# PJLab-ADG/neuralsim

Hardware: AMD Instinct MI355X
Metric: training rays/sec (fwd+bwd) NeuS 800x800 (higher is better)
Workload: dtype fp16

## Files before the change

neuralsim_amd/csrc/field.hip:

```cpp
#include "lotd_dev.h"
#include "mfma_mlp.h"
#include "occ_dev.h"
#include <stdlib.h>

enum { M_W1 = 0, M_W2, M_W2T, M_W1T, M_R1, M_R2, M_R3, M_R3T, M_R2T, M_R1T, M_COUNT };
enum { V_B1 = 0, V_B2, V_WH, V_RB1, V_RB2, V_RB3, V_SCAL, V_COUNT };

struct FieldLayout {
  int64_t mat[M_COUNT];
  int64_t vec[V_COUNT];
  int64_t vend;
  int64_t mat16[4];
  int64_t total;
  int elt;
  int split;
};

static const int kMatUo[M_COUNT] = {64, 64, 64, 32, 64, 64, 32, 64, 64, 32};
static const int kMatUi[M_COUNT] = {32, 64, 64, 64, 32, 64, 64, 32, 64, 64};

static inline int mat_uo(int m, int nc) { return m == M_W1T ? 32 * nc : kMatUo[m]; }
static inline int mat_ui(int m, int nc) { return m == M_W1 ? 32 * nc : kMatUi[m]; }
static inline int field_nc(int num_levels) { return num_levels > 16 ? 2 : 1; }
static inline int field_ne(const NsimFieldMeta* meta) { return meta->embed_E > 0 ? 2 : 0; }
// ... 439 lines not shown
#pragma unroll
        for (int b = 0; b < 2; ++b) {
          const int l = 4 * q + 2 * hi + b, r0 = 4 * q + 2 * b;
          const float* hp = reinterpret_cast<const float*>(pf + 256 * l) + 2 * j;
          h[r0] = valid ? hp[0] : 0.f;
          h[r0 + 1] = valid ? hp[1] : 0.f;
        }
      nsim_wait_lgkm0();
      p = load_point(a, tile, j, true);
      const int64_t sc = valid ? s : a.S - 1;
#pragma unroll
      for (int q = 0; q < 4; ++q)
#pragma unroll
        for (int b = 0; b < 2; ++b) {
          const int l = 4 * q + 2 * hi + b, r0 = 4 * q + 2 * b;
          const JPair<JT>* jp = reinterpret_cast<const JPair<JT>*>(reinterpret_cast<const JT*>(a.J_pl) + ((int64_t)l * a.PS + sc) * 6);
          Jq[2 * q + b][0] = jp[0];
          Jq[2 * q + b][1] = jp[1];
          Jq[2 * q + b][2] = jp[2];
        }
      if (tile + wstride < ntiles) prefetch_planes(tile + wstride);
    } else if constexpr (GLDS) {
      nsim_wait_vm0();
#pragma unroll
      for (int m = 0; m < NC; ++m)
#pragma unroll
      for (int q = 0; q < 4; ++q)
#pragma unroll
        for (int b = 0; b < 2; ++b) {
          const int l = 16 * m + 4 * q + 2 * hi + b, r0 = 16 * m + 4 * q + 2 * b;
          const float* hp = reinterpret_cast<const float*>(pf + 1024 * l) + 2 * j;
          const JT* jp = reinterpret_cast<const JT*>(pf + 1024 * l + 256) + 6 * j;
          const bool lv = valid && LV_OK(l);
          h[r0] = lv ? hp[0] : 0.f;
          h[r0 + 1] = lv ? hp[1] : 0.f;
          float ja[3], jb[3];
          jload6(jp, ja, jb);
#pragma unroll
          for (int c3 = 0; c3 < 3; ++c3) {
            J[r0][c3] = lv ? ja[c3] : 0.f;
            J[r0 + 1][c3] = lv ? jb[c3] : 0.f;
          }
        }
      nsim_wait_lgkm0();
      if (tile + wstride < ntiles) prefetch_planes(tile + wstride);
    } else if constexpr (FROM_PLANES) {
#pragma unroll
      for (int m = 0; m < NC; ++m)
#pragma unroll
        for (int q = 0; q < 4; ++q)
#pragma unroll
          for (int b = 0; b < 2; ++b) {
            const int l = 16 * m + 4 * q + 2 * hi + b;
            const int r0 = 16 * m + 4 * q + 2 * b;
            h[r0] = h[r0 + 1] = 0.f;
            if (valid && LV_OK(l)) {
              const float* hp = a.h_pl + ((int64_t)l * a.PS + s) * 2;
              h[r0] = hp[0];
              h[r0 + 1] = hp[1];
            }
          }
      if constexpr (NC == 1 && NE == 0) {
#pragma unroll
        for (int q = 0; q < 4; ++q)
#pragma unroll
          for (int b = 0; b < 2; ++b) {
            const int l = 4 * q + 2 * hi + b;
            const int r0 = 4 * q + 2 * b;
#pragma unroll
            for (int c3 = 0; c3 < 3; ++c3) J[r0][c3] = J[r0 + 1][c3] = 0.f;
            if (valid && LV_OK(l)) {
              jload6(reinterpret_cast<const JT*>(a.J_pl) + ((int64_t)l * a.PS + s) * 6, J[r0], J[r0 + 1]);
            }
          }
      }
    } else if constexpr (NC == 1) {
#pragma unroll
      for (int q = 0; q < 4; ++q) {
#pragma unroll
        for (int b = 0; b < 2; ++b) {
          const int l = 4 * q + 2 * hi + b;
          const LotdRes R = a.lotd.res[l];
          const LotdCell c = lotd_cell(p.xx, R, a.lotd);
          float f0 = 0.f, f1 = 0.f, j0[3] = {0.f, 0.f, 0.f}, j1[3] = {0.f, 0.f, 0.f};
          const int pm = lotd_slot_mask(c);
          if (l < a.lotd.n_active)
#pragma unroll
          for (int slot = 0; slot < 8; ++slot) {
            const int corner = slot ^ pm;
            float w, dw[3];
            lotd_corner_w(c, corner, w, dw);
            const uint32_t idx = lotd_index(c.c0[0] + (corner & 1), c.c0[1] + ((corner >> 1) & 1),
                                            c.c0[2] + ((corner >> 2) & 1), R, a.lotd.type[l], a.lotd.size[l]);
            float g0, g1;
            lotd_load2(gref, (uint32_t)a.lotd.offset[l] + p.goff + 2u * idx, g0, g1);
            f0 = f0 + w * g0;
            f1 = f1 + w * g1;
#pragma unroll
            for (int c3 = 0; c3 < 3; ++c3) {
              j0[c3] = j0[c3] + dw[c3] * g0;
              j1[c3] = j1[c3] + dw[c3] * g1;
            }
          }
          const int r0 = 4 * q + 2 * b;
          h[r0] = f0;
          h[r0 + 1] = f1;
#pragma unroll
          for (int c3 = 0; c3 < 3; ++c3) {
            J[r0][c3] = j0[c3] * c.dscale[c3];
            J[r0 + 1][c3] = j1[c3] * c.dscale[c3];
          }
          if (a.h_pl && valid) {
            float* hp = a.h_pl + ((int64_t)l * a.PS + s) * 2;
            JT* jp = reinterpret_cast<JT*>(a.J_pl) + ((int64_t)l * a.PS + s) * 6;
            hp[0] = f0;
            hp[1] = f1;
            jstore6(jp, J[r0], J[r0 + 1]);
          }
        }
      }
    }
    if constexpr (NE > 0) embed_eval(a, p.xx, valid, hi, reinterpret_cast<float(&)[32]>(h[16 * NC]), ed);
    float a1[32];
    dense<PREC, 2, NI>(a1, W + L.mat[M_W1], h, true);
#pragma unroll
    for (int k = 0; k < 32; ++k) a1[k] = softplus_b(a1[k] + vecf(W, L, V_B1, hi, k), beta, inv_beta);
    float a2[32];
    if constexpr (SDF_D == 2) {
      dense<PREC, 2, 2>(a2, W + L.mat[M_W2], a1, false);
#pragma unroll
      for (int k = 0; k < 32; ++k) a2[k] = softplus_b(a2[k] + vecf(W, L, V_B2, hi, k), beta, inv_beta);
    } else {
#pragma unroll
      for (int k = 0; k < 32; ++k) a2[k] = a1[k];
    }
    float sdf = 0.f;
#pragma unroll
    for (int k = 0; k < 32; ++k) sdf = sdf + vecf(W, L, V_WH, hi, k) * a2[k];
    sdf = sdf + wave_shfl_xor(sdf, 32);
    sdf = sdf + b_out;
    float e1[32];
    float d1[32];
    if constexpr (SDF_D == 2) {
      float d2[32];
#pragma unroll
      for (int k = 0; k < 32; ++k) d2[k] = sig_from_softplus(a2[k], beta) * vecf(W, L, V_WH, hi, k);
      dense<PREC, 2, 2>(e1, W + L.mat[M_W2T], d2, false);
#pragma unroll
      for (int k = 0; k < 32; ++k) d1[k] = sig_from_softplus(a1[k], beta) * e1[k];
    } else {
#pragma unroll
      for (int k = 0; k < 32; ++k) {
        e1[k] = vecf(W, L, V_WH, hi, k);
        d1[k] = sig_from_softplus(a1[k], beta) * e1[k];
      }
    }
    float g[16 * NI];
    dense<PREC, NI, 2>(g, W + L.mat[M_W1T], d1, false);
    float nab[3];
    if constexpr (JDIR) {
      float acc[3] = {0.f, 0.f, 0.f};
#pragma unroll
      for (int e = 0; e < 8; ++e) {
        const int r0 = 4 * (e >> 1) + 2 * (e & 1);
        acc[0] = acc[0] + g[r0] * (float)Jq[e][0].x + g[r0 + 1] * (float)Jq[e][1].y;
        acc[1] = acc[1] + g[r0] * (float)Jq[e][0].y + g[r0 + 1] * (float)Jq[e][2].x;
        acc[2] = acc[2] + g[r0] * (float)Jq[e][1].x + g[r0 + 1] * (float)Jq[e][2].y;
      }
#pragma unroll
      for (int c3 = 0; c3 < 3; ++c3) nab[c3] = acc[c3] + wave_shfl_xor(acc[c3], 32);
    } else if constexpr ((NC == 1 && NE == 0) || GL2) {
#pragma unroll
      for (int c3 = 0; c3 < 3; ++c3) {
        float acc = 0.f;
#pragma unroll
        for (int f = 0; f < 16 * NC; ++f) acc = acc + g[f] * J[f][c3];
        nab[c3] = acc + wave_shfl_xor(acc, 32);
      }
    } else {
      float acc[3] = {0.f, 0.f, 0.f};
      if (valid) {
#pragma unroll
        for (int m = 0; m < NC; ++m)
#pragma unroll
          for (int q = 0; q < 4; ++q)
// ... 591 lines not shown
        dz1[k] = gs * wh * s1 + dh1[k] * wh * (beta * s1 * (1.0f - s1));
      }
    }
    bh += wave_sum(g == 0 ? gs : 0.f);
    __syncthreads();
    jstage16<4>(stA, dz1, wave);
    jstage16<2>(stB, h, wave);
    if constexpr (SDF_D == 1) jstage16<4>(stC, whv, wave);
    __syncthreads();
    if (do_dw) {
      jdw16_tiles<2>(stA, wave, stB, 0, accW1, &bs1);
      if constexpr (SDF_D == 1) bsh += j16_row_share(stC, wave);
    }
    float dh[8];
    dense16<2, 4>(dh, W + L.mat16[M_W1T], dz1, true);
    if (a.dx) {
      float acc[3] = {0.f, 0.f, 0.f};
      if (valid) {
#pragma unroll
        for (int m = 0; m < 2; ++m)
#pragma unroll
          for (int b = 0; b < 2; ++b) {
            const int l = 8 * m + 2 * g + b, r0 = 4 * m + 2 * b;
            float ja[3], jb[3];
            jload6(reinterpret_cast<const JT*>(a.J_pl) + ((int64_t)l * a.PS + s) * 6, ja, jb);
#pragma unroll
            for (int c3 = 0; c3 < 3; ++c3) acc[c3] = acc[c3] + dh[r0] * ja[c3] + dh[r0 + 1] * jb[c3];
          }
      }
#pragma unroll
      for (int c3 = 0; c3 < 3; ++c3) {
        acc[c3] = acc[c3] + wave_shfl_xor(acc[c3], 16);
        acc[c3] = acc[c3] + wave_shfl_xor(acc[c3], 32);
      }
      if (valid && g == 0) {
#pragma unroll
        for (int c3 = 0; c3 < 3; ++c3) a.dx[3 * s + c3] = a.dx[3 * s + c3] + acc[c3];
      }
    }
    if (valid && a.dh_pl) {
#pragma unroll
      for (int m = 0; m < 2; ++m)
#pragma unroll
        for (int b = 0; b < 2; ++b) {
          const int l = 8 * m + 2 * g + b, r0 = 4 * m + 2 * b;
          float* dp = a.dh_pl + ((int64_t)l * a.S + s) * 2;
          dp[0] = dh[r0];
          dp[1] = dh[r0 + 1];
        }
    }
  }
  const int F1 = 2 * a.lotd.num_levels;
  const SrcOff so = src_off(SDF_D, F1);
  const int64_t ro = (int64_t)(blockIdx.x & (unsigned)a.rep_mask) * a.rep_stride;
#pragma unroll
  for (int n = 0; n < 2; ++n) jflush16(a.dsdf_w + ro + so.w1, F1, F1, wave, n, accW1[n]);
  bs1 += wave_shfl_xor(bs1, 16);
  bs1 += wave_shfl_xor(bs1, 32);
  bsh += wave_shfl_xor(bsh, 16);
  bsh += wave_shfl_xor(bsh, 32);
  if constexpr (SDF_D == 2) {
#pragma unroll
    for (int n = 0; n < 4; ++n) jflush16(a.dsdf_w + ro + so.w2, 64, 64, wave, n, accW2[n]);
    bs2 += wave_shfl_xor(bs2, 16);
    bs2 += wave_shfl_xor(bs2, 32);
    if (g == 0 && bs2 != 0.f) atomicAdd(&a.dsdf_b[ro + so.b2 + 16 * wave + p], bs2);
  }
  if (g == 0 && bs1 != 0.f) atomicAdd(&a.dsdf_b[ro + so.b1 + 16 * wave + p], bs1);
  if (g == 0 && bsh != 0.f) atomicAdd(&a.dsdf_w[ro + so.wh + 16 * wave + p], bsh);
  if (lane == 0 && bh != 0.f) atomicAdd(&a.dsdf_b[ro + so.bh], bh);
}

#define SDF_H_SCALE 1024.0f
#ifndef NSIM_SDF_MIN_WAVES
#define NSIM_SDF_MIN_WAVES 2
#endif
constexpr int GLM_PTS = 2;
constexpr int GLM_PTS_WJ = 1;
template <int PREC, bool WJ>
__global__ void __launch_bounds__(64, 1) k_lotd_gather_lm(FieldArgs a) {
  using JT = typename JPlane<PREC>::T;
  constexpr int NP = WJ ? GLM_PTS_WJ : GLM_PTS;
  const int lane = nsim_lane();
  const int xcd = (int)(blockIdx.x & 7u);
  const int64_t s0 = (int64_t)(blockIdx.x >> 3) * (64 * NP) + lane;
  int64_t Sv = a.S;
  if (a.S_dev) {
    const int64_t sd = a.S_dev[0] + a.S_add;
    Sv = sd <= Sv ? sd : 0;
  }
  if (s0 - lane >= Sv) return;
  float xx[NP][3];
  uint32_t goff[NP];
#pragma unroll
  for (int q = 0; q < NP; ++q) {
    const int64_t s = s0 + 64 * q;
    xx[q][0] = xx[q][1] = xx[q][2] = 0.f;
    goff[q] = 0u;
    if (s < Sv) {
      if (a.ray_goff) goff[q] = (uint32_t)a.ray_goff[a.ridx[s]];
      if (a.x) {
        xx[q][0] = a.x[3 * s]; xx[q][1] = a.x[3 * s + 1]; xx[q][2] = a.x[3 * s + 2];
      } else {
        const int64_t ray = a.ridx[s];
        const float tt = a.t[s];
#pragma unroll
        for (int c = 0; c < 3; ++c) xx[q][c] = a.rays_o[3 * ray + c] + tt * a.rays_d[3 * ray + c];
      }
    }
  }
  const GridRef gref = grid_ref(a.grid);
  const int nl = a.glm_n[xcd];
  const int64_t nblk_valid = (Sv + 64 * NP - 1) / (64 * NP);
  const bool second_half = (int64_t)(blockIdx.x >> 3) >= (nblk_valid + 1) / 2;
#pragma unroll 1
  for (int k = 0; k < nl; ++k) {
    const int l = a.glm_lv[xcd][k];
    const int half = a.glm_half[xcd][k];
    if ((half == 1 && second_half) || (half == 2 && !second_half)) continue;
    const LotdRes R = a.lotd.res[l];
    const int type = a.lotd.type[l];
    const uint32_t T = a.lotd.size[l], off = (uint32_t)a.lotd.offset[l];
    float f0[NP], f1[NP];
    float j0[WJ ? NP : 1][3], j1[WJ ? NP : 1][3];
#pragma unroll
    for (int q = 0; q < NP; ++q) {
      const LotdCell c = lotd_cell(xx[q], R, a.lotd);
      f0[q] = f1[q] = 0.f;
      if constexpr (WJ) {
#pragma unroll
        for (int c3 = 0; c3 < 3; ++c3) j0[q][c3] = j1[q][c3] = 0.f;
      }
      constexpr bool SLOTS = WJ;
      const LotdSlots SL = lotd_slots(c);
      const int pm = lotd_slot_mask(c);
      if (l < a.lotd.n_active)
#pragma unroll
      for (int slot = 0; slot < 8; ++slot) {
        float w, dw[3];
        uint32_t idx;
        if constexpr (SLOTS) {
          lotd_slot_w(SL, slot, w, dw);
          idx = lotd_slot_index(SL, slot, R, type, T);
        } else {
          const int corner = slot ^ pm;
          lotd_corner_w(c, corner, w, dw);
          idx = lotd_index(c.c0[0] + (corner & 1), c.c0[1] + ((corner >> 1) & 1), c.c0[2] + ((corner >> 2) & 1), R, type, T);
        }
        float g0, g1;
        lotd_load2(gref, off + goff[q] + 2u * idx, g0, g1);
        f0[q] = f0[q] + w * g0;
        f1[q] = f1[q] + w * g1;
        if constexpr (WJ) {
#pragma unroll
          for (int c3 = 0; c3 < 3; ++c3) {
            j0[q][c3] = j0[q][c3] + dw[c3] * g0;
            j1[q][c3] = j1[q][c3] + dw[c3] * g1;
          }
        }
      }
      if constexpr (WJ) {
#pragma unroll
        for (int c3 = 0; c3 < 3; ++c3) {
          j0[q][c3] = j0[q][c3] * c.dscale[c3];
          j1[q][c3] = j1[q][c3] * c.dscale[c3];
        }
      }
    }
#pragma unroll
    for (int q = 0; q < NP; ++q) {
      const int64_t s = s0 + 64 * q;
      if (s < Sv) {
        const int64_t e = (int64_t)l * a.PS + s;
        if constexpr (WJ) {
          const int64_t ep = (int64_t)l * a.PS + s;
          float* hp = a.h_pl + ep * 2;
          JT* jp = reinterpret_cast<JT*>(a.J_pl) + ep * 6;
          hp[0] = f0[q];
          hp[1] = f1[q];
          jstore6(jp, j0[q], j1[q]);
        } else if constexpr (PREC == 0) {
          union {
            uint32_t u;
            f16 h[2];
          } cv;
          cv.h[0] = (f16)f16_sat(f0[q] * SDF_H_SCALE);
          cv.h[1] = (f16)f16_sat(f1[q] * SDF_H_SCALE);
          reinterpret_cast<uint32_t*>(a.feat_pl)[e] = cv.u;
        } else {
          reinterpret_cast<float*>(a.feat_pl)[2 * e] = f0[q];
          reinterpret_cast<float*>(a.feat_pl)[2 * e + 1] = f1[q];
        }
      }
    }
  }
}

template <int PREC, bool WJ>
static void launch_gather_lm(const FieldArgs& a, int64_t S, hipStream_t stream) {
  const dim3 gg((unsigned)(8 * nsim_blocks(S, 64 * (WJ ? GLM_PTS_WJ : GLM_PTS))));
  hipLaunchKernelGGL((k_lotd_gather_lm<PREC, WJ>), gg, dim3(64), 0, stream, a);
}

__device__ __forceinline__ void sdf_gather8(const FieldArgs& a, const GridRef& gref, const TilePoint& p, int lb, int hi,
                                            float (&f8)[8]) {
#pragma unroll
  for (int qq = 0; qq < 2; ++qq) {
#pragma unroll
    for (int b = 0; b < 2; ++b) {
      const int l = lb + 4 * qq + 2 * hi + b;
      const LotdRes R = a.lotd.res[l];
      const LotdCell c = lotd_cell(p.xx, R, a.lotd);
      float f0 = 0.f, f1 = 0.f;
      const int pm = lotd_slot_mask(c);
      if (l < a.lotd.n_active)
#pragma unroll
      for (int slot = 0; slot < 8; ++slot) {
        const int corner = slot ^ pm;
        float w, dw[3];
        lotd_corner_w(c, corner, w, dw);
        const uint32_t idx = lotd_index(c.c0[0] + (corner & 1), c.c0[1] + ((corner >> 1) & 1),
                                        c.c0[2] + ((corner >> 2) & 1), R, a.lotd.type[l], a.lotd.size[l]);
        float g0, g1;
        lotd_load2(gref, (uint32_t)a.lotd.offset[l] + p.goff + 2u * idx, g0, g1);
        f0 = f0 + w * g0;
        f1 = f1 + w * g1;
      }
      f8[4 * qq + 2 * b] = f0;
      f8[4 * qq + 2 * b + 1] = f1;
    }
  }
}

template <int PREC, int NC, bool HAVE_BV>
__device__ __forceinline__ void sdf_layer1_step(const char* W, const FieldLayout& L, int rb, int lane, const float (&f8)[8],
                                                const f16x8& bvp, f32x16 (&acc)[2], f32x16 (&accc)[PREC == 2 ? 2 : 1]) {
  constexpr bool PLANES = HAVE_BV;
  if constexpr (PREC == 0) {
    f16x8 bv;
    if constexpr (PLANES) {
      bv = bvp;
    } else {
#pragma unroll
      for (int e = 0; e < 8; ++e) bv[e] = (f16)f16_sat(f8[e] * SDF_H_SCALE);
    }
    const f16x8* A = reinterpret_cast<const f16x8*>(W + L.mat[M_W1]);
#pragma unroll
    for (int mo = 0; mo < 2; ++mo) acc[mo] = mfma_32x32x16_f16(A[(mo * 2 * NC + rb) * 64 + lane], bv, acc[mo]);
  } else if constexpr (PREC == 2) {
    f16x8 bh, bl;
#pragma unroll
    for (int e = 0; e < 8; ++e) {
      f16 h_, l_;
      split_f16(f8[e] * SDF_H_SCALE, h_, l_);
      bh[e] = h_;
      bl[e] = l_;
    }
    const f16x8* Ah = reinterpret_cast<const f16x8*>(W + L.mat[M_W1]);
    const f16x8* Al = Ah + 64 * 4 * NC;
#pragma unroll
    for (int mo = 0; mo < 2; ++mo) {
      const int fi = (mo * 2 * NC + rb) * 64 + lane;
      acc[mo] = mfma_32x32x16_f16(Ah[fi], bh, acc[mo]);
      accc[mo] = mfma_32x32x16_f16(Ah[fi], bl, accc[mo]);
      accc[mo] = mfma_32x32x16_f16(Al[fi], bh, accc[mo]);
    }
  } else {
    const float* A = reinterpret_cast<const float*>(W + L.mat[M_W1]);
#pragma unroll
    for (int e = 0; e < 8; ++e)
#pragma unroll
      for (int mo = 0; mo < 2; ++mo)
        acc[mo] = mfma_32x32x2_f32(A[(mo * 16 * NC + 8 * rb + e) * 64 + lane], f8[e], acc[mo]);
  }
}

template <int PREC, int SDF_D>
__device__ __forceinline__ float sdf_decode(const char* W, const FieldLayout& L, f32x16 (&acc)[2],
                                            f32x16 (&accc)[PREC == 2 ? 2 : 1], int hi, int lane, float beta, float inv_beta,
                                            float b_out) {
  const float inv_h = PREC != 1 ? 1.0f / SDF_H_SCALE : 1.0f;
  float sdf = 0.f;
  if constexpr (PREC == 2) {
#pragma unroll
    for (int mo = 0; mo < 2; ++mo)
#pragma unroll
      for (int r = 0; r < 16; ++r) acc[mo][r] = acc[mo][r] + accc[mo][r] * (1.0f / SPLIT_LO_SCALE);
  }
  if constexpr (PREC == 2 && SDF_D == 2) {
    f16x8 bqh[4], bql[4];
#pragma unroll
    for (int mo = 0; mo < 2; ++mo)
#pragma unroll
      for (int r = 0; r < 16; ++r) {
        f16 h_, l_;
        split_f16(softplus_exact(acc[mo][r] * inv_h + vecf(W, L, V_B1, hi, mo * 16 + r), beta, inv_beta), h_, l_);
        bqh[2 * mo + (r >> 3)][r & 7] = h_;
        bql[2 * mo + (r >> 3)][r & 7] = l_;
      }
    const f16x8* A2h = reinterpret_cast<const f16x8*>(W + L.mat[M_W2]);
    const f16x8* A2l = A2h + 64 * 8;
#pragma unroll
    for (int mo = 0; mo < 2; ++mo) {
      f32x16 acc2 = zero16(), acc2c = zero16();
#pragma unroll
      for (int st = 0; st < 4; ++st) {
        const int fi = (mo * 4 + st) * 64 + lane;
        acc2 = mfma_32x32x16_f16(A2h[fi], bqh[st], acc2);
        acc2c = mfma_32x32x16_f16(A2h[fi], bql[st], acc2c);
        acc2c = mfma_32x32x16_f16(A2l[fi], bqh[st], acc2c);
      }
#pragma unroll
// ... 1326 lines not shown
```

neuralsim_amd/csrc/lotd.hip:

```cpp
#include "lotd_dev.h"

__global__ void __launch_bounds__(256) k_lotd_fwd(const float* __restrict__ x, const f16* __restrict__ grid,
                                                   LotdDev m, int64_t S, float* __restrict__ out,
                                                   float* __restrict__ dydx) {
  const int64_t tid = (int64_t)blockIdx.x * blockDim.x + threadIdx.x;
  const int L = m.num_levels;
  if (tid >= S * L) return;
  const int64_t s = tid / L;
  const int l = (int)(tid % L);
  const float xx[3] = {x[3 * s], x[3 * s + 1], x[3 * s + 2]};
  const LotdRes R = m.res[l];
  const LotdCell c = lotd_cell(xx, R, m);
  float f0 = 0.f, f1 = 0.f;
  float j0[3] = {0.f, 0.f, 0.f}, j1[3] = {0.f, 0.f, 0.f};
  const int pm = lotd_slot_mask(c);
  if (l < m.n_active)
#pragma unroll
  for (int slot = 0; slot < 8; ++slot) {
    const int corner = slot ^ pm;
    float w, dw[3];
    lotd_corner_w(c, corner, w, dw);
    const uint32_t idx = lotd_index(c.c0[0] + (corner & 1), c.c0[1] + ((corner >> 1) & 1),
                                    c.c0[2] + ((corner >> 2) & 1), R, m.type[l], m.size[l]);
    float g0, g1;
    lotd_load2(grid, m.offset[l], idx, g0, g1);
    f0 = f0 + w * g0;
    f1 = f1 + w * g1;
    if (dydx) {
#pragma unroll
      for (int a = 0; a < 3; ++a) {
        j0[a] = j0[a] + dw[a] * g0;
        j1[a] = j1[a] + dw[a] * g1;
      }
    }
  }
  const int64_t o = s * (2 * L) + 2 * l;
  out[o] = f0;
  out[o + 1] = f1;
  if (dydx) {
#pragma unroll
    for (int a = 0; a < 3; ++a) {
      dydx[o * 3 + a] = j0[a] * c.dscale[a];
      dydx[(o + 1) * 3 + a] = j1[a] * c.dscale[a];
    }
  }
}

__global__ void __launch_bounds__(256) k_lotd_bwd(const float* __restrict__ x, const float* __restrict__ dout,
                                                   const float* __restrict__ ddydx, LotdDev m, int64_t S,
                                                   float* __restrict__ dgrid) {
  const int64_t tid = (int64_t)blockIdx.x * blockDim.x + threadIdx.x;
  const int L = m.num_levels;
  if (tid >= S * L) return;
  const int64_t s = tid / L;
  const int l = (int)(tid % L);
  if (l >= m.n_active) return;
  const float xx[3] = {x[3 * s], x[3 * s + 1], x[3 * s + 2]};
  const LotdRes R = m.res[l];
  const LotdCell c = lotd_cell(xx, R, m);
  const int64_t o = s * (2 * L) + 2 * l;
  const float d0 = dout ? dout[o] : 0.f, d1 = dout ? dout[o + 1] : 0.f;
  float q0[3] = {0.f, 0.f, 0.f}, q1[3] = {0.f, 0.f, 0.f};
  if (ddydx) {
#pragma unroll
    for (int a = 0; a < 3; ++a) {
      q0[a] = ddydx[o * 3 + a] * c.dscale[a];
      q1[a] = ddydx[(o + 1) * 3 + a] * c.dscale[a];
    }
  }
#pragma unroll
  for (int corner = 0; corner < 8; ++corner) {
    float w, dw[3];
    lotd_corner_w(c, corner, w, dw);
    const uint32_t idx = lotd_index(c.c0[0] + (corner & 1), c.c0[1] + ((corner >> 1) & 1),
                                    c.c0[2] + ((corner >> 2) & 1), R, m.type[l], m.size[l]);
    const float v0 = w * d0 + (dw[0] * q0[0] + dw[1] * q0[1] + dw[2] * q0[2]);
    const float v1 = w * d1 + (dw[0] * q1[0] + dw[1] * q1[1] + dw[2] * q1[2]);
    float* dst = dgrid + m.offset[l] + 2 * (int64_t)idx;
    if (v0 != 0.f) atomicAdd(dst, v0);
    if (v1 != 0.f) atomicAdd(dst + 1, v1);
  }
}

extern "C" {

int nsim_lotd_fwd(const float* x, const void* grid_f16, const NsimLotdMeta* meta, int64_t S, float* out,
                  float* dydx, void* stream) {
  const int rc = lotd_meta_check(meta);
  if (rc) return rc;
  if (S <= 0) return 0;
  hipLaunchKernelGGL(k_lotd_fwd, dim3(nsim_blocks(S * meta->num_levels, 256)), dim3(256), 0, (hipStream_t)stream, x,
                     (const f16*)grid_f16, lotd_dev(meta), S, out, dydx);
  NSIM_CHECK_LAUNCH();
  return 0;
}

int nsim_lotd_bwd(const float* x, const float* dL_dout, const float* dL_ddydx, const NsimLotdMeta* meta, int64_t S,
                  float* dgrid, void* stream) {
  const int rc = lotd_meta_check(meta);
  if (rc) return rc;
  if (S <= 0) return 0;
  hipLaunchKernelGGL(k_lotd_bwd, dim3(nsim_blocks(S * meta->num_levels, 256)), dim3(256), 0, (hipStream_t)stream, x,
                     dL_dout, dL_ddydx, lotd_dev(meta), S, dgrid);
  NSIM_CHECK_LAUNCH();
  return 0;
}

}
```

neuralsim_amd/csrc/lotd_dev.h:

```cpp
#pragma once
#include "nsim_common.h"

struct LotdRes {
  int r[3];
  __host__ __device__ int max() const { return r[0] > r[1] ? (r[0] > r[2] ? r[0] : r[2]) : (r[1] > r[2] ? r[1] : r[2]); }
};

struct LotdDev {
  int num_levels;
  int n_active;
  LotdRes res[NSIM_MAX_LEVELS];
  int type[NSIM_MAX_LEVELS];
  uint32_t size[NSIM_MAX_LEVELS];
  int64_t offset[NSIM_MAX_LEVELS];
  float xs[3], xb[3];
};

static inline LotdDev lotd_dev(const NsimLotdMeta* m) {
  LotdDev d;
  d.num_levels = m->num_levels;
  d.n_active = (m->n_active_levels > 0 && m->n_active_levels < m->num_levels) ? m->n_active_levels : m->num_levels;
  for (int l = 0; l < NSIM_MAX_LEVELS; ++l) {
    for (int a = 0; a < 3; ++a) d.res[l].r[a] = l < m->num_levels ? m->res[l][a] : 2;
    d.type[l] = l < m->num_levels ? m->type[l] : 0;
    d.size[l] = l < m->num_levels ? m->size[l] : 8;
    d.offset[l] = l < m->num_levels ? m->offset[l] : 0;
  }
  const bool unit = m->x_scale[0] == 0.f && m->x_scale[1] == 0.f && m->x_scale[2] == 0.f;
  for (int a = 0; a < 3; ++a) {
    d.xs[a] = unit ? 0.5f : m->x_scale[a];
    d.xb[a] = unit ? 0.5f : m->x_shift[a];
  }
  return d;
}

static inline int lotd_meta_check(const NsimLotdMeta* m) {
  if (!m) return 10;
  if (m->n_feats != 2) return 11;
  if (m->num_levels < 1 || m->num_levels > NSIM_MAX_LEVELS) return 12;
  for (int l = 0; l < m->num_levels; ++l) {
    if (m->res[l][0] < 2 || m->res[l][1] < 2 || m->res[l][2] < 2) return 13;
    if (m->type[l] == NSIM_LOTD_DENSE) {
      if ((uint64_t)m->res[l][0] * m->res[l][1] * m->res[l][2] != (uint64_t)m->size[l]) return 14;
    } else if (m->type[l] == NSIM_LOTD_HASH) {
      if (m->size[l] == 0 || (m->size[l] & (m->size[l] - 1)) != 0) return 17;
    } else {
      return 15;
    }
    if (m->offset[l] & 1) return 16;
  }
  return 0;
}

struct LotdCell {
  int c0[3];
  float w[3];
  float dscale[3];
};

__device__ __forceinline__ LotdCell lotd_cell(const float x[3], const LotdRes& R, const LotdDev& L) {
  LotdCell c;
#pragma unroll
  for (int a = 0; a < 3; ++a) {
    const float rm1 = (float)(R.r[a] - 1);
    const float u = x[a] * L.xs[a] + L.xb[a];
    const float pos = u * rm1;
    float f = floorf(pos);
    f = fminf(fmaxf(f, 0.f), (float)(R.r[a] - 2));
    c.c0[a] = (int)f;
    c.w[a] = pos - f;
    c.dscale[a] = L.xs[a] * rm1;
  }
  return c;
}

__device__ __forceinline__ uint32_t lotd_index(int cx, int cy, int cz, const LotdRes& R, int type, uint32_t T) {
  if (type == NSIM_LOTD_DENSE)
    return (uint32_t)cx + (uint32_t)R.r[0] * ((uint32_t)cy + (uint32_t)R.r[1] * (uint32_t)cz);
  const uint32_t h = (uint32_t)cx ^ ((uint32_t)cy * 2654435761u) ^ ((uint32_t)cz * 805459861u);
  return h & (T - 1u);
}

__device__ __forceinline__ int lotd_slot_mask(const LotdCell& c) {
  return NSIM_GATHER_PARITY ? ((c.c0[0] & 1) | ((c.c0[1] & 1) << 1) | ((c.c0[2] & 1) << 2)) : 0;
}

struct LotdSlots {
  int v[3][2];
  float w[3][2];
  float s[3];
};
__device__ __forceinline__ LotdSlots lotd_slots(const LotdCell& c) {
  LotdSlots S;
#pragma unroll
  for (int a = 0; a < 3; ++a) {
    const int p = NSIM_GATHER_PARITY ? (c.c0[a] & 1) : 0;
    S.v[a][0] = c.c0[a] + p;
    S.v[a][1] = c.c0[a] + (p ^ 1);
    const float w1 = c.w[a], w0 = 1.0f - c.w[a];
    S.w[a][0] = p ? w1 : w0;
    S.w[a][1] = p ? w0 : w1;
    S.s[a] = p ? 1.0f : -1.0f;
  }
  return S;
}
__device__ __forceinline__ void lotd_slot_w(const LotdSlots& S, int k, float& w, float dw[3]) {
  const int kx = k & 1, ky = (k >> 1) & 1, kz = (k >> 2) & 1;
  const float wx = S.w[0][kx], wy = S.w[1][ky], wz = S.w[2][kz];
  const float wxy = wx * wy;
  w = wxy * wz;
  dw[0] = (kx ? -S.s[0] : S.s[0]) * (wy * wz);
  dw[1] = (ky ? -S.s[1] : S.s[1]) * (wx * wz);
  dw[2] = (kz ? -S.s[2] : S.s[2]) * wxy;
}
__device__ __forceinline__ uint32_t lotd_slot_index(const LotdSlots& S, int k, const LotdRes& R, int type, uint32_t T) {
  return lotd_index(S.v[0][k & 1], S.v[1][(k >> 1) & 1], S.v[2][(k >> 2) & 1], R, type, T);
}

__device__ __forceinline__ void lotd_corner_w(const LotdCell& c, int corner, float& w, float dw[3]) {
  const int dx = corner & 1, dy = (corner >> 1) & 1, dz = (corner >> 2) & 1;
  const float wx = dx ? c.w[0] : 1.0f - c.w[0];
  const float wy = dy ? c.w[1] : 1.0f - c.w[1];
  const float wz = dz ? c.w[2] : 1.0f - c.w[2];
  w = wx * wy * wz;
  dw[0] = (dx ? 1.0f : -1.0f) * wy * wz;
  dw[1] = (dy ? 1.0f : -1.0f) * wx * wz;
  dw[2] = (dz ? 1.0f : -1.0f) * wx * wy;
}

__device__ __forceinline__ void lotd_load2(const f16* grid, int64_t off, uint32_t idx, float& f0, float& f1) {
  const uint32_t raw = *reinterpret_cast<const uint32_t*>(grid + off + 2 * (int64_t)idx);
  union {
    uint32_t u;
    f16 h[2];
  } cv;
  cv.u = raw;
  f0 = (float)cv.h[0];
  f1 = (float)cv.h[1];
}


__device__ __forceinline__ void lotd_load2(const GridRef& g, uint32_t elem_off, float& f0, float& f1) {
  union {
    uint32_t u;
    f16 h[2];
  } cv;
  cv.u = grid_load_u32(g, elem_off);
  f0 = (float)cv.h[0];
  f1 = (float)cv.h[1];
}
```

neuralsim_amd/csrc/nsim_prims.h:

```cpp
#pragma once
#include <hip/hip_runtime.h>

#define NSIM_DYN_SMEM(name) extern __shared__ __attribute__((aligned(16))) char name[]

__device__ __forceinline__ int nsim_lane() { return (int)(threadIdx.x & 63); }

template <class T>
__device__ __forceinline__ T wave_shfl(T v, int src) {
  return __shfl(v, src, 64);
}

__device__ __forceinline__ unsigned long long wave_ballot(int pred) { return __ballot(pred); }

template <int I, class T>
__device__ __forceinline__ T quad_bcast(T v) {
  static_assert(sizeof(T) == 4, "quad_bcast: 32-bit types only");
  int iv;
  __builtin_memcpy(&iv, &v, 4);
  iv = __builtin_amdgcn_update_dpp(0, iv, I | (I << 2) | (I << 4) | (I << 6), 0xf, 0xf, true);
  T r;
  __builtin_memcpy(&r, &iv, 4);
  return r;
}

#define NSIM_DPP_OLD_F32(oldv, x, ctrl, rmask)                                                              \
  __builtin_bit_cast(float, __builtin_amdgcn_update_dpp(__builtin_bit_cast(int, (float)(oldv)),             \
                                                        __builtin_bit_cast(int, (x)), (ctrl), (rmask), 0xf, false))
#define NSIM_DPP_F32(x, ctrl) \
  __builtin_bit_cast(float, __builtin_amdgcn_update_dpp(0, __builtin_bit_cast(int, (x)), (ctrl), 0xf, 0xf, true))

__device__ __forceinline__ float nsim_readlane_f32(float v, int l) {
  return __builtin_bit_cast(float, __builtin_amdgcn_readlane(__builtin_bit_cast(int, v), l));
}

__device__ __forceinline__ float wave_incl_sum(float v) {
  v += NSIM_DPP_OLD_F32(0.f, v, 0x111, 0xf);
  v += NSIM_DPP_OLD_F32(0.f, v, 0x112, 0xf);
  v += NSIM_DPP_OLD_F32(0.f, v, 0x114, 0xf);
  v += NSIM_DPP_OLD_F32(0.f, v, 0x118, 0xf);
  v += NSIM_DPP_OLD_F32(0.f, v, 0x142, 0xa);
  v += NSIM_DPP_OLD_F32(0.f, v, 0x143, 0xc);
  return v;
}

#define NSIM_DPP_OLD_I32(oldv, x, ctrl, rmask) __builtin_amdgcn_update_dpp((int)(oldv), (int)(x), (ctrl), (rmask), 0xf, false)
__device__ __forceinline__ int wave_incl_sum(int v) {
  v += NSIM_DPP_OLD_I32(0, v, 0x111, 0xf);
  v += NSIM_DPP_OLD_I32(0, v, 0x112, 0xf);
  v += NSIM_DPP_OLD_I32(0, v, 0x114, 0xf);
  v += NSIM_DPP_OLD_I32(0, v, 0x118, 0xf);
  v += NSIM_DPP_OLD_I32(0, v, 0x142, 0xa);
  v += NSIM_DPP_OLD_I32(0, v, 0x143, 0xc);
  return v;
}

__device__ __forceinline__ int64_t wave_incl_sum(int64_t v) {
  uint32_t lo = (uint32_t)(uint64_t)v, hi = (uint32_t)((uint64_t)v >> 32);
#define NSIM_SCAN64_STEP(ctrl, rmask)                                  \
  {                                                                    \
    const uint32_t sl = (uint32_t)NSIM_DPP_OLD_I32(0, lo, ctrl, rmask); \
    const uint32_t sh = (uint32_t)NSIM_DPP_OLD_I32(0, hi, ctrl, rmask); \
    const uint32_t nl = lo + sl;                                       \
    hi = hi + sh + (nl < lo ? 1u : 0u);                                \
    lo = nl;                                                           \
  }
  NSIM_SCAN64_STEP(0x111, 0xf)
  NSIM_SCAN64_STEP(0x112, 0xf)
  NSIM_SCAN64_STEP(0x114, 0xf)
  NSIM_SCAN64_STEP(0x118, 0xf)
  NSIM_SCAN64_STEP(0x142, 0xa)
  NSIM_SCAN64_STEP(0x143, 0xc)
#undef NSIM_SCAN64_STEP
  return (int64_t)(((uint64_t)hi << 32) | (uint64_t)lo);
}

__device__ __forceinline__ float wave_incl_prod(float v) {
  v *= NSIM_DPP_OLD_F32(1.f, v, 0x111, 0xf);
  v *= NSIM_DPP_OLD_F32(1.f, v, 0x112, 0xf);
  v *= NSIM_DPP_OLD_F32(1.f, v, 0x114, 0xf);
  v *= NSIM_DPP_OLD_F32(1.f, v, 0x118, 0xf);
  v *= NSIM_DPP_OLD_F32(1.f, v, 0x142, 0xa);
  v *= NSIM_DPP_OLD_F32(1.f, v, 0x143, 0xc);
  return v;
}

__device__ __forceinline__ float wave_sum(float v) {
  v += NSIM_DPP_F32(v, 0xB1);
  v += NSIM_DPP_F32(v, 0x4E);
  v += NSIM_DPP_F32(v, 0x141);
  v += NSIM_DPP_F32(v, 0x140);
  return (nsim_readlane_f32(v, 0) + nsim_readlane_f32(v, 16)) + (nsim_readlane_f32(v, 32) + nsim_readlane_f32(v, 48));
}

__device__ __forceinline__ float wave_max(float v) {
  v = fmaxf(v, NSIM_DPP_F32(v, 0xB1));
  v = fmaxf(v, NSIM_DPP_F32(v, 0x4E));
  v = fmaxf(v, NSIM_DPP_F32(v, 0x141));
  v = fmaxf(v, NSIM_DPP_F32(v, 0x140));
  return fmaxf(fmaxf(nsim_readlane_f32(v, 0), nsim_readlane_f32(v, 16)),
               fmaxf(nsim_readlane_f32(v, 32), nsim_readlane_f32(v, 48)));
}

__device__ __forceinline__ void wave_sync_lds() {
  __builtin_amdgcn_fence(__ATOMIC_RELEASE, "wavefront");
  __builtin_amdgcn_wave_barrier();
  __builtin_amdgcn_fence(__ATOMIC_ACQUIRE, "wavefront");
}
__device__ __forceinline__ void nsim_release_agent() {
  __builtin_amdgcn_fence(__ATOMIC_RELEASE, "agent");
  asm volatile("s_waitcnt vmcnt(0)" ::: "memory");
}
__device__ __forceinline__ void nsim_wave_fence() { __threadfence_block(); }
// ... 75 lines not shown
```

Measured before the change: 7.163 million.

## Pair adjacent lanes to split trilinear corner gathers in LoTD gather kernel

In the non-Jacobian gather kernel, each pair of adjacent lanes now exchanges sample positions via DPP swizzle and each lane fetches four of the eight corners for both points, with x-parity flipped per lane, then combines partial sums with a lane-xor shuffle. The goal is to make neighbouring lanes hit adjacent grid addresses for better coalescing and cache-line locality. Separately, the corner accumulations in several trilinear loops are split into two independent accumulators to shorten FMA dependency chains. It costs extra shuffles and cell computations per lane and changes the floating-point summation order.

```diff
diff --git a/neuralsim_amd/csrc/field.hip b/neuralsim_amd/csrc/field.hip
--- a/neuralsim_amd/csrc/field.hip
+++ b/neuralsim_amd/csrc/field.hip
@@ -545,7 +545,7 @@
           const int l = 4 * q + 2 * hi + b;
           const LotdRes R = a.lotd.res[l];
           const LotdCell c = lotd_cell(p.xx, R, a.lotd);
-          float f0 = 0.f, f1 = 0.f, j0[3] = {0.f, 0.f, 0.f}, j1[3] = {0.f, 0.f, 0.f};
+          float fa[2] = {0.f, 0.f}, fb[2] = {0.f, 0.f}, ja[2][3] = {{0.f, 0.f, 0.f}, {0.f, 0.f, 0.f}}, jb[2][3] = {{0.f, 0.f, 0.f}, {0.f, 0.f, 0.f}};
           const int pm = lotd_slot_mask(c);
           if (l < a.lotd.n_active)
 #pragma unroll
@@ -557,13 +557,20 @@
                                             c.c0[2] + ((corner >> 2) & 1), R, a.lotd.type[l], a.lotd.size[l]);
             float g0, g1;
             lotd_load2(gref, (uint32_t)a.lotd.offset[l] + p.goff + 2u * idx, g0, g1);
-            f0 = f0 + w * g0;
-            f1 = f1 + w * g1;
+            fa[slot & 1] = fa[slot & 1] + w * g0;
+            fb[slot & 1] = fb[slot & 1] + w * g1;
 #pragma unroll
             for (int c3 = 0; c3 < 3; ++c3) {
-              j0[c3] = j0[c3] + dw[c3] * g0;
-              j1[c3] = j1[c3] + dw[c3] * g1;
+              ja[slot & 1][c3] = ja[slot & 1][c3] + dw[c3] * g0;
+              jb[slot & 1][c3] = jb[slot & 1][c3] + dw[c3] * g1;
             }
+          }
+          const float f0 = fa[0] + fa[1], f1 = fb[0] + fb[1];
+          float j0[3], j1[3];
+#pragma unroll
+          for (int c3 = 0; c3 < 3; ++c3) {
+            j0[c3] = ja[0][c3] + ja[1][c3];
+            j1[c3] = jb[0][c3] + jb[1][c3];
           }
           const int r0 = 4 * q + 2 * b;
           h[r0] = f0;
@@ -1321,6 +1328,9 @@
   using JT = typename JPlane<PREC>::T;
   constexpr int NP = WJ ? GLM_PTS_WJ : GLM_PTS;
   const int lane = nsim_lane();
+  constexpr bool PAIR = !WJ;
+  constexpr int PP = PAIR ? 2 : 1;
+  const int h = PAIR ? (lane & 1) : 0;
   const int xcd = (int)(blockIdx.x & 7u);
   const int64_t s0 = (int64_t)(blockIdx.x >> 3) * (64 * NP) + lane;
   int64_t Sv = a.S;
@@ -1329,23 +1339,38 @@
     Sv = sd <= Sv ? sd : 0;
   }
   if (s0 - lane >= Sv) return;
-  float xx[NP][3];
-  uint32_t goff[NP];
+  float xx[NP][PP][3];
+  uint32_t goff[NP][PP];
 #pragma unroll
   for (int q = 0; q < NP; ++q) {
     const int64_t s = s0 + 64 * q;
-    xx[q][0] = xx[q][1] = xx[q][2] = 0.f;
-    goff[q] = 0u;
+    float xo[3] = {0.f, 0.f, 0.f};
+    uint32_t go = 0u;
     if (s < Sv) {
-      if (a.ray_goff) goff[q] = (uint32_t)a.ray_goff[a.ridx[s]];
+      if (a.ray_goff) go = (uint32_t)a.ray_goff[a.ridx[s]];
       if (a.x) {
-        xx[q][0] = a.x[3 * s]; xx[q][1] = a.x[3 * s + 1]; xx[q][2] = a.x[3 * s + 2];
+        xo[0] = a.x[3 * s]; xo[1] = a.x[3 * s + 1]; xo[2] = a.x[3 * s + 2];
       } else {
         const int64_t ray = a.ridx[s];
         const float tt = a.t[s];
 #pragma unroll
-        for (int c = 0; c < 3; ++c) xx[q][c] = a.rays_o[3 * ray + c] + tt * a.rays_d[3 * ray + c];
-      }
+        for (int c = 0; c < 3; ++c) xo[c] = a.rays_o[3 * ray + c] + tt * a.rays_d[3 * ray + c];
+      }
+    }
+    if constexpr (PAIR) {
+      const uint32_t gp = wave_shfl_xor(go, 1);
+      goff[q][0] = h ? gp : go;
+      goff[q][PP - 1] = h ? go : gp;
+#pragma unroll
+      for (int c = 0; c < 3; ++c) {
+        const float xp = wave_shfl_xor(xo[c], 1);
+        xx[q][0][c] = h ? xp : xo[c];
+        xx[q][PP - 1][c] = h ? xo[c] : xp;
+      }
+    } else {
+      goff[q][0] = go;
+#pragma unroll
+      for (int c = 0; c < 3; ++c) xx[q][0][c] = xo[c];
     }
   }
   const GridRef gref = grid_ref(a.grid);
@@ -1360,75 +1385,85 @@
     const LotdRes R = a.lotd.res[l];
     const int type = a.lotd.type[l];
     const uint32_t T = a.lotd.size[l], off = (uint32_t)a.lotd.offset[l];
-    float f0[NP], f1[NP];
-    float j0[WJ ? NP : 1][3], j1[WJ ? NP : 1][3];
+    float f0[NP][2], f1[NP][2];
+    float j0[WJ ? NP : 1][2][3], j1[WJ ? NP : 1][2][3];
 #pragma unroll
     for (int q = 0; q < NP; ++q) {
-      const LotdCell c = lotd_cell(xx[q], R, a.lotd);
-      f0[q] = f1[q] = 0.f;
-      if constexpr (WJ) {
-#pragma unroll
-        for (int c3 = 0; c3 < 3; ++c3) j0[q][c3] = j1[q][c3] = 0.f;
-      }
-      constexpr bool SLOTS = WJ;
-      const LotdSlots SL = lotd_slots(c);
-      const int pm = lotd_slot_mask(c);
-      if (l < a.lotd.n_active)
-#pragma unroll
-      for (int slot = 0; slot < 8; ++slot) {
-        float w, dw[3];
-        uint32_t idx;
-        if constexpr (SLOTS) {
+#pragma unroll
+      for (int i = 0; i < 2; ++i) {
+        f0[q][i] = f1[q][i] = 0.f;
+        if constexpr (WJ) {
+#pragma unroll
+          for (int c3 = 0; c3 < 3; ++c3) j0[q][i][c3] = j1[q][i][c3] = 0.f;
+        }
+      }
+#pragma unroll
+      for (int p = 0; p < PP; ++p) {
+        const LotdCell c = lotd_cell(xx[q][p], R, a.lotd);
+        const LotdSlots SL = lotd_slots(c, h);
+        if (l < a.lotd.n_active)
+#pragma unroll
+        for (int slot = 0; slot < 8; slot += PP) {
+          const int i = PAIR ? p : (slot & 1);
+          float w, dw[3];
           lotd_slot_w(SL, slot, w, dw);
-          idx = lotd_slot_index(SL, slot, R, type, T);
-        } else {
-          const int corner = slot ^ pm;
-          lotd_corner_w(c, corner, w, dw);
-          idx = lotd_index(c.c0[0] + (corner & 1), c.c0[1] + ((corner >> 1) & 1), c.c0[2] + ((corner >> 2) & 1), R, type, T);
-        }
-        float g0, g1;
-        lotd_load2(gref, off + goff[q] + 2u * idx, g0, g1);
-        f0[q] = f0[q] + w * g0;
-        f1[q] = f1[q] + w * g1;
-        if constexpr (WJ) {
-#pragma unroll
-          for (int c3 = 0; c3 < 3; ++c3) {
-            j0[q][c3] = j0[q][c3] + dw[c3] * g0;
-            j1[q][c3] = j1[q][c3] + dw[c3] * g1;
+          const uint32_t idx = lotd_slot_index(SL, slot, R, type, T);
+          float g0, g1;
+          lotd_load2(gref, off + goff[q][p] + 2u * idx, g0, g1);
+          f0[q][i] = f0[q][i] + w * g0;
+          f1[q][i] = f1[q][i] + w * g1;
+          if constexpr (WJ) {
+#pragma unroll
+            for (int c3 = 0; c3 < 3; ++c3) {
+              j0[q][i][c3] = j0[q][i][c3] + dw[c3] * g0;
+              j1[q][i][c3] = j1[q][i][c3] + dw[c3] * g1;
+            }
           }
         }
       }
+    }
+    float dscale[3];
+#pragma unroll
+    for (int c3 = 0; c3 < 3; ++c3) dscale[c3] = a.lotd.xs[c3] * (float)(R.r[c3] - 1);
+    auto pair_sum = [h](float p0, float p1) {
+      if constexpr (PAIR) {
+        const float got = wave_shfl_xor(h ? p0 : p1, 1);
+        return h ? got + p1 : p0 + got;
+      } else {
+        return p0 + p1;
+      }
+    };
+#pragma unroll
+    for (int q = 0; q < NP; ++q) {
+      const float F0 = pair_sum(f0[q][0], f0[q][1]), F1 = pair_sum(f1[q][0], f1[q][1]);
+      float J0[3], J1[3];
       if constexpr (WJ) {
 #pragma unroll
         for (int c3 = 0; c3 < 3; ++c3) {
-          j0[q][c3] = j0[q][c3] * c.dscale[c3];
-          j1[q][c3] = j1[q][c3] * c.dscale[c3];
+          J0[c3] = pair_sum(j0[q][0][c3], j0[q][1][c3]) * dscale[c3];
+          J1[c3] = pair_sum(j1[q][0][c3], j1[q][1][c3]) * dscale[c3];
         }
       }
-    }
-#pragma unroll
-    for (int q = 0; q < NP; ++q) {
       const int64_t s = s0 + 64 * q;
       if (s < Sv) {
         const int64_t e = (int64_t)l * a.PS + s;
         if constexpr (WJ) {
-          const int64_t ep = (int64_t)l * a.PS + s;
-          float* hp = a.h_pl + ep * 2;
-          JT* jp = reinterpret_cast<JT*>(a.J_pl) + ep * 6;
-          hp[0] = f0[q];
-          hp[1] = f1[q];
-          jstore6(jp, j0[q], j1[q]);
+          float* hp = a.h_pl + e * 2;
+          JT* jp = reinterpret_cast<JT*>(a.J_pl) + e * 6;
+          hp[0] = F0;
+          hp[1] = F1;
+          jstore6(jp, J0, J1);
         } else if constexpr (PREC == 0) {
           union {
             uint32_t u;
             f16 h[2];
           } cv;
-          cv.h[0] = (f16)f16_sat(f0[q] * SDF_H_SCALE);
-          cv.h[1] = (f16)f16_sat(f1[q] * SDF_H_SCALE);
+          cv.h[0] = (f16)f16_sat(F0 * SDF_H_SCALE);
+          cv.h[1] = (f16)f16_sat(F1 * SDF_H_SCALE);
           reinterpret_cast<uint32_t*>(a.feat_pl)[e] = cv.u;
         } else {
-          reinterpret_cast<float*>(a.feat_pl)[2 * e] = f0[q];
-          reinterpret_cast<float*>(a.feat_pl)[2 * e + 1] = f1[q];
+          reinterpret_cast<float*>(a.feat_pl)[2 * e] = F0;
+          reinterpret_cast<float*>(a.feat_pl)[2 * e + 1] = F1;
         }
       }
     }
@@ -1450,7 +1485,7 @@
       const int l = lb + 4 * qq + 2 * hi + b;
       const LotdRes R = a.lotd.res[l];
       const LotdCell c = lotd_cell(p.xx, R, a.lotd);
-      float f0 = 0.f, f1 = 0.f;
+      float f0[2] = {0.f, 0.f}, f1[2] = {0.f, 0.f};
       const int pm = lotd_slot_mask(c);
       if (l < a.lotd.n_active)
 #pragma unroll
@@ -1462,11 +1497,11 @@
                                         c.c0[2] + ((corner >> 2) & 1), R, a.lotd.type[l], a.lotd.size[l]);
         float g0, g1;
         lotd_load2(gref, (uint32_t)a.lotd.offset[l] + p.goff + 2u * idx, g0, g1);
-        f0 = f0 + w * g0;
-        f1 = f1 + w * g1;
-      }
-      f8[4 * qq + 2 * b] = f0;
-      f8[4 * qq + 2 * b + 1] = f1;
+        f0[slot & 1] = f0[slot & 1] + w * g0;
+        f1[slot & 1] = f1[slot & 1] + w * g1;
+      }
+      f8[4 * qq + 2 * b] = f0[0] + f0[1];
+      f8[4 * qq + 2 * b + 1] = f1[0] + f1[1];
     }
   }
 }
diff --git a/neuralsim_amd/csrc/lotd.hip b/neuralsim_amd/csrc/lotd.hip
--- a/neuralsim_amd/csrc/lotd.hip
+++ b/neuralsim_amd/csrc/lotd.hip
@@ -11,8 +11,8 @@
   const float xx[3] = {x[3 * s], x[3 * s + 1], x[3 * s + 2]};
   const LotdRes R = m.res[l];
   const LotdCell c = lotd_cell(xx, R, m);
-  float f0 = 0.f, f1 = 0.f;
-  float j0[3] = {0.f, 0.f, 0.f}, j1[3] = {0.f, 0.f, 0.f};
+  float fa[2] = {0.f, 0.f}, fb[2] = {0.f, 0.f};
+  float ja[2][3] = {{0.f, 0.f, 0.f}, {0.f, 0.f, 0.f}}, jb[2][3] = {{0.f, 0.f, 0.f}, {0.f, 0.f, 0.f}};
   const int pm = lotd_slot_mask(c);
   if (l < m.n_active)
 #pragma unroll
@@ -24,15 +24,22 @@
                                     c.c0[2] + ((corner >> 2) & 1), R, m.type[l], m.size[l]);
     float g0, g1;
     lotd_load2(grid, m.offset[l], idx, g0, g1);
-    f0 = f0 + w * g0;
-    f1 = f1 + w * g1;
+    fa[slot & 1] = fa[slot & 1] + w * g0;
+    fb[slot & 1] = fb[slot & 1] + w * g1;
     if (dydx) {
 #pragma unroll
       for (int a = 0; a < 3; ++a) {
-        j0[a] = j0[a] + dw[a] * g0;
-        j1[a] = j1[a] + dw[a] * g1;
+        ja[slot & 1][a] = ja[slot & 1][a] + dw[a] * g0;
+        jb[slot & 1][a] = jb[slot & 1][a] + dw[a] * g1;
       }
     }
+  }
+  const float f0 = fa[0] + fa[1], f1 = fb[0] + fb[1];
+  float j0[3], j1[3];
+#pragma unroll
+  for (int a = 0; a < 3; ++a) {
+    j0[a] = ja[0][a] + ja[1][a];
+    j1[a] = jb[0][a] + jb[1][a];
   }
   const int64_t o = s * (2 * L) + 2 * l;
   out[o] = f0;
diff --git a/neuralsim_amd/csrc/lotd_dev.h b/neuralsim_amd/csrc/lotd_dev.h
--- a/neuralsim_amd/csrc/lotd_dev.h
+++ b/neuralsim_amd/csrc/lotd_dev.h
@@ -90,11 +90,11 @@
   float w[3][2];
   float s[3];
 };
-__device__ __forceinline__ LotdSlots lotd_slots(const LotdCell& c) {
+__device__ __forceinline__ LotdSlots lotd_slots(const LotdCell& c, int hx = 0) {
   LotdSlots S;
 #pragma unroll
   for (int a = 0; a < 3; ++a) {
-    const int p = NSIM_GATHER_PARITY ? (c.c0[a] & 1) : 0;
+    const int p = (NSIM_GATHER_PARITY ? (c.c0[a] & 1) : 0) ^ (a == 0 ? hx : 0);
     S.v[a][0] = c.c0[a] + p;
     S.v[a][1] = c.c0[a] + (p ^ 1);
     const float w1 = c.w[a], w0 = 1.0f - c.w[a];
diff --git a/neuralsim_amd/csrc/nsim_prims.h b/neuralsim_amd/csrc/nsim_prims.h
--- a/neuralsim_amd/csrc/nsim_prims.h
+++ b/neuralsim_amd/csrc/nsim_prims.h
@@ -28,6 +28,14 @@
                                                         __builtin_bit_cast(int, (x)), (ctrl), (rmask), 0xf, false))
 #define NSIM_DPP_F32(x, ctrl) \
   __builtin_bit_cast(float, __builtin_amdgcn_update_dpp(0, __builtin_bit_cast(int, (x)), (ctrl), 0xf, 0xf, true))
+
+__device__ __forceinline__ float wave_shfl_xor(float v, int mask) {
+  if (__builtin_constant_p(mask) && mask == 1) return NSIM_DPP_F32(v, 0xB1);
+  return wave_shfl(v, nsim_lane() ^ mask);
+}
+__device__ __forceinline__ uint32_t wave_shfl_xor(uint32_t v, int mask) {
+  return __builtin_bit_cast(uint32_t, wave_shfl_xor(__builtin_bit_cast(float, v), mask));
+}
 
 __device__ __forceinline__ float nsim_readlane_f32(float v, int l) {
   return __builtin_bit_cast(float, __builtin_amdgcn_readlane(__builtin_bit_cast(int, v), l));
```

Result: faster. 7.271 million, median of 6 (+1.5%).
